# zhanglei1172/sam-quantization

Hardware: AMD Instinct MI355X
Metric: 1024×1024 images/sec through quantized ViT-H encoder; % of MFMA/HBM roofline (higher is better)
Workload: dtype fp16

## Files before the change

### sam-quantization_amd/csrc/attention.hip

```cpp
#include "common.h"

#include <cstdio>
#include <cstdlib>
#include <algorithm>
#include <string>
#include <type_traits>
#include <vector>

namespace samq {

constexpr float LOG2E = 1.4426950408889634f;

__device__ __attribute__((aligned(16))) _Float16 g_zero16[8];

struct AttnParams {
  const _Float16* qkv;
  const _Float16* qkv_bias;
  const _Float16* relh;
  const _Float16* relw;
  _Float16* out;
  int64_t tok_stride;
  int C, heads;
  int S;
  int H, W;
// ... 100 lines not shown
    const _Float16* src = g_zero16;
    bool real = false;
    if (c < UNIT_CHUNKS) {
      constexpr int HALF = UNIT_CHUNKS / 2;
      const bool isv = c >= HALF;
      const int cc = isv ? c - HALF : c;
      const int key = cc / D8, d8 = cc % D8;
      const int r = RESIDENT ? key / S : 0;
      const int slot = RESIDENT ? key % S : key;
      const int kind = r < S ? tok_kind(r, slot) : 2;
      const int off = (isv ? 2 * C : C) + head * D + d8 * 8;
      if (kind == 0) { src = tok_ptr(r, slot) + off; real = true; }
      else if (kind == 1 && p.qkv_bias) src = p.qkv_bias + off;
    }
    src0[i] = src;
    adv[i] = real && !RESIDENT;
  }
  const int64_t rowstride = (int64_t)p.W * p.tok_stride;
  auto issue = [&](int row0, int buf) {
#pragma unroll
    for (int i = 0; i < NI; ++i) {
      const _Float16* src = adv[i] ? src0[i] + row0 * rowstride : src0[i];
      __builtin_amdgcn_global_load_lds((const SAMQ_GLOBAL void*)src,
                                       (SAMQ_LDS void*)(smem + buf * BUFB + (wave * NI + i) * 1024), 16, 0, 0);
    }
  };

  issue(0, 0);
  if (!RESIDENT && S > 1) issue(1, 1);

  const bool kin3 = 64 + 8 * g < D;
  half8_t qf[QT][KS];
  int qrow[QT], qcol0[QT];
#pragma unroll
  for (int t = 0; t < QT; ++t) {
    const int qi = (qblk * NW + wave) * QT + t;
    qrow[t] = qi / KT;
    qcol0[t] = (qi % KT) * 16;
    const int kind = tok_kind(qrow[t], qcol0[t] + ql);
    const _Float16* src = nullptr;
    if (kind == 0) src = tok_ptr(qrow[t], qcol0[t] + ql) + head * D;
    else if (kind == 1 && p.qkv_bias) src = p.qkv_bias + head * D;
#pragma unroll
    for (int s = 0; s < KS; ++s) {
      half8_t v = {};
      if (src && (s < 2 || kin3)) v = *(const half8_t*)(src + 32 * s + 8 * g);
#pragma unroll
      for (int j = 0; j < 8; ++j) v[j] = (_Float16)((float)v[j] * qscale);
      qf[t][s] = v;
    }
  }

  float4_t tw[QT][KT];
  const float inv_scale = 1.0f / p.scale;
  float* th_w = th_lds + wave * (QT * TH_ROWS * 16);
#pragma unroll
  for (int t = 0; t < QT; ++t) {
    const int qh = qrow[t] < S ? qrow[t] : S - 1;
    if (!PRECOMP) {
#pragma unroll
      for (int which = 0; which < 2; ++which) {
        const _Float16* tab = which ? p.relw : p.relh;
#pragma unroll
        for (int kt = 0; kt < KT; ++kt) {
          int r = qh - (kt * 16 + ql) + S - 1;
          r = r < 0 ? 0 : r;
          const _Float16* rp = tab + (int64_t)r * D;
          float4_t a = {0.f, 0.f, 0.f, 0.f};
#pragma unroll
          for (int s = 0; s < KS; ++s) {
            half8_t ra = {};
            if (s < 2 || kin3) ra = *(const half8_t*)(rp + 32 * s + 8 * g);
            a = __builtin_amdgcn_mfma_f32_16x16x32_f16(ra, qf[t][s], a, 0, 0, 0);
          }
          a = a * inv_scale;
          if (which) {
            tw[t][kt] = a;
          } else {
#pragma unroll
            for (int r2 = 0; r2 < 4; ++r2) th_w[(t * TH_ROWS + kt * 16 + 4 * g + r2) * 16 + ql] = a[r2];
          }
        }
      }
    } else {
      const int qw = qcol0[t] + ql;
      const bool ok = qw < S && qrow[t] < S;
      const int64_t base = ((((int64_t)unit * p.heads + head) * S + qh) * S + (ok ? qw : 0)) * S;
#pragma unroll
      for (int kt = 0; kt < KT; ++kt) {
#pragma unroll
        for (int r2 = 0; r2 < 4; ++r2) {
          const int kk = kt * 16 + 4 * g + r2;
          const bool kin = ok && kk < S;
          tw[t][kt][r2] = kin ? (float)p.relw[base + kk] * LOG2E : 0.f;
          th_w[(t * TH_ROWS + kk) * 16 + ql] = kin ? (float)p.relh[base + kk] * LOG2E : 0.f;
        }
      }
    }
  }

  constexpr bool MSUM = SP >= 32;
  float m[QT], l[QT];
  float4_t o[QT][DT], lacc[QT];
  const half8_t ones = {1, 1, 1, 1, 1, 1, 1, 1};
#pragma unroll
  for (int t = 0; t < QT; ++t) {
    m[t] = -INFINITY;
    l[t] = 0.f;
    lacc[t] = float4_t{0.f, 0.f, 0.f, 0.f};
#pragma unroll
    for (int d = 0; d < DT; ++d) o[t][d] = float4_t{0.f, 0.f, 0.f, 0.f};
  }
  const bool mask_slots = S < SP;
  const int trow = ql >> 2;
  const int tcol = 4 * (ql & 3);

  if (RESIDENT) {
    wait_vmcnt<0>();
    __syncthreads();
  } else {
    __syncthreads();
  }

  using PB = half8_t[QT][(SP + 31) / 32];
  auto qk = [&](const char* kb, float4_t (&sc)[QT][KT]) {
#pragma unroll
      for (int kt = 0; kt < KT; ++kt) {
        const char* krow = kb + (kt * 16 + ql) * (D * 2);
        half8_t kf[KS];
#pragma unroll
        for (int s = 0; s < KS; ++s) kf[s] = *(const half8_t*)(krow + (32 * s + 8 * g) * 2);
#pragma unroll
        for (int t = 0; t < QT; ++t) {
          float4_t a = tw[t][kt];
#pragma unroll
          for (int s = 0; s < KS; ++s) a = __builtin_amdgcn_mfma_f32_16x16x32_f16(kf[s], qf[t][s], a, 0, 0, 0);
          sc[t][kt] = a;
        }
      }

  };
  auto soft = [&](int kh, float4_t (&sc)[QT][KT], PB& pb, half4_t (&pb16)[QT]) {
    bool any_rescale = false;
    float alpha[QT];
#pragma unroll
    for (int t = 0; t < QT; ++t) {
      if (mask_slots) {
#pragma unroll
        for (int kt = 0; kt < KT; ++kt)
#pragma unroll
          for (int r = 0; r < 4; ++r)
            if (kt * 16 + 4 * g + r >= S) sc[t][kt][r] = -INFINITY;
      }
      float mx;
      if constexpr (KT == 1) {
        mx = max3f(sc[t][0][0], sc[t][0][1], fmaxf(sc[t][0][2], sc[t][0][3]));
      } else {
        mx = max3f(sc[t][0][0], sc[t][0][1], sc[t][0][2]);
        float my = max3f(sc[t][1][0], sc[t][1][1], sc[t][1][2]);
        mx = max3f(mx, sc[t][0][3], sc[t][1][3]);
#pragma unroll
        for (int kt = 2; kt < KT; kt += 2) {
          mx = max3f(mx, sc[t][kt][0], sc[t][kt][1]);
          my = max3f(my, sc[t][kt + 1][0], sc[t][kt + 1][1]);
          mx = max3f(mx, sc[t][kt][2], sc[t][kt][3]);
          my = max3f(my, sc[t][kt + 1][2], sc[t][kt + 1][3]);
        }
        mx = fmaxf(mx, my);
      }
      mx = max_rows4(mx);
      const float th = th_w[(t * TH_ROWS + kh) * 16 + ql];
      const float mrow = mx + th;
      const bool up = mrow > m[t] + 8.0f;
      const float mnew = up ? mrow : m[t];
      alpha[t] = up ? __builtin_amdgcn_exp2f(m[t] - mnew) : 1.0f;
      any_rescale |= up;
      m[t] = mnew;
      const float corr = mnew - th;
      float rs = 0.f;
#pragma unroll
      for (int kt = 0; kt < KT; ++kt)
#pragma unroll
        for (int r = 0; r < 4; ++r) {
          const float e = __builtin_amdgcn_exp2f(sc[t][kt][r] - corr);
          sc[t][kt][r] = e;
          if (!MSUM) rs += e;
        }
      if (!MSUM) l[t] = l[t] * alpha[t] + rs;
      if (SP == 16) {
        pb16[t] = half4_t{(_Float16)sc[t][0][0], (_Float16)sc[t][0][1], (_Float16)sc[t][0][2], (_Float16)sc[t][0][3]};
      } else {
#pragma unroll
        for (int s = 0; s < SP / 32; ++s) {
#pragma unroll
          for (int r = 0; r < 4; ++r) {
            pb[t][s][r] = (_Float16)sc[t][2 * s][r];
            pb[t][s][4 + r] = (_Float16)sc[t][2 * s + 1][r];
          }
        }
      }
    }
    if (__any(any_rescale)) {
#pragma unroll
      for (int t = 0; t < QT; ++t)
#pragma unroll
        for (int d = 0; d < DT; ++d) o[t][d] = o[t][d] * alpha[t];
#pragma unroll
      for (int t = 0; t < QT; ++t)
        if (MSUM) lacc[t] = lacc[t] * alpha[t];
    }

  };
  auto pv = [&](const char* vb, PB& pb, half4_t (&pb16)[QT]) {
    const uint32_t vbase = lds_addr(vb + ((4 * g + trow) * D + tcol) * 2);
    static_for<DT>([&](auto dc_) {
      constexpr int d = decltype(dc_)::value;
      if constexpr (SP == 16) {
        half4_t va = ds_read_tr16_off<(d * 16) * 2>(vbase);
        asm volatile("s_waitcnt lgkmcnt(0)" : "+v"(va));
#pragma unroll
        for (int t = 0; t < QT; ++t) o[t][d] = __builtin_amdgcn_mfma_f32_16x16x16f16(va, pb16[t], o[t][d], 0, 0, 0);
      } else {
        constexpr int NS = SP / 32;
        half4_t lo[NS], hi[NS];
        static_for<NS>([&](auto sc_) {
          constexpr int s_ = decltype(sc_)::value;
          lo[s_] = ds_read_tr16_off<((32 * s_) * D + d * 16) * 2>(vbase);
          hi[s_] = ds_read_tr16_off<((32 * s_ + 16) * D + d * 16) * 2>(vbase);
        });
        if constexpr (NS == 2) {
          asm volatile("s_waitcnt lgkmcnt(0)" : "+v"(lo[0]), "+v"(hi[0]), "+v"(lo[1]), "+v"(hi[1]));
        } else {
#pragma unroll
          for (int s = 0; s < NS; ++s) asm volatile("s_waitcnt lgkmcnt(0)" : "+v"(lo[s]), "+v"(hi[s]));
        }
#pragma unroll
        for (int s = 0; s < NS; ++s) {
          const half8_t va = {lo[s][0], lo[s][1], lo[s][2], lo[s][3], hi[s][0], hi[s][1], hi[s][2], hi[s][3]};
#pragma unroll
          for (int t = 0; t < QT; ++t) o[t][d] = __builtin_amdgcn_mfma_f32_16x16x32_f16(va, pb[t][s], o[t][d], 0, 0, 0);
        }
      }
    });
    if constexpr (MSUM) {
      constexpr int NS = SP / 32;
#pragma unroll
      for (int s = 0; s < NS; ++s)
#pragma unroll
        for (int t = 0; t < QT; ++t) lacc[t] = __builtin_amdgcn_mfma_f32_16x16x32_f16(ones, pb[t][s], lacc[t], 0, 0, 0);
    }
  };

  if (RESIDENT) {
    for (int kh = 0; kh < S; ++kh) {
      const char* kb = smem + kh * S * (D * 2);
      float4_t sc[QT][KT];
      PB pb;
      half4_t pb16[QT];
      qk(kb, sc);
      soft(kh, sc, pb, pb16);
      pv(kb + (UNIT_CHUNKS / 2) * 16, pb, pb16);
    }
  } else {
    float4_t scA[QT][KT], scB[QT][KT];
    PB pb;
    half4_t pb16[QT];
    if (S > 1) wait_vmcnt<NI>(); else wait_vmcnt<0>();
    __builtin_amdgcn_s_barrier();
    qk(smem, scA);
    auto step = [&](int kh, float4_t (&cur)[QT][KT], float4_t (&nxt)[QT][KT]) {
      if (kh + 1 < S) {
        wait_vmcnt<0>();
        __builtin_amdgcn_s_barrier();
        if (kh + 2 < S) issue(kh + 2, (kh + 2) % 3);
        qk(smem + ((kh + 1) % 3) * BUFB, nxt);
      }
      soft(kh, cur, pb, pb16);
      pv(smem + (kh % 3) * BUFB + ROWB, pb, pb16);
    };
    for (int kh = 0; kh < S; kh += 2) {
      step(kh, scA, scB);
      step(kh + 1, scB, scA);
    }
  }

#pragma unroll
  for (int t = 0; t < QT; ++t) {
    float lt = l[t];
    if (MSUM) {
      lt = lacc[t][0];
    } else {
      lt += __shfl_xor(lt, 16, 64);
      lt += __shfl_xor(lt, 32, 64);
    }
    const int x = qcol0[t] + ql;
    if (tok_kind(qrow[t], x) != 0) continue;
    const float inv = 1.0f / lt;
    const int64_t dst = (((int64_t)b * p.H + (Y0 + qrow[t])) * p.W + (X0 + x)) * C + head * D;
#pragma unroll
    for (int d = 0; d < DT; ++d) attn_store4(p, dst + d * 16 + 4 * g, o[t][d] * inv);
  }
}

template <int D, bool UNSC = false, bool PHL = false>
struct Win {
  static constexpr int S = 14, QT = 2;
  static constexpr int KS = D == 80 ? 3 : 2;
  static constexpr int DT = D / 16;
  static constexpr int NPC = D == 80 ? 5 : 4;
  static constexpr int ROWB = NPC * 1024;
  static constexpr int KVB = S * ROWB;
  static constexpr int V0 = (NPC - 2) * 1024;
  static constexpr int TAB = (2 * S - 1) * D;
  static constexpr int TABB = ((2 * TAB * 2 + 1023) / 1024) * 1024;
  static_assert(D == 64 || D == 80, "head dim");

  struct Geo { const _Float16* tok0; int b, Y0, X0, head, nrow, ncol; };

  __device__ static __forceinline__ Geo geo(const AttnParams& p, int item) {
    Geo o;
    const int unit = item / p.heads;
    o.head = item - unit * p.heads;
    o.b = unit / p.upi;
    const int wi = unit - o.b * p.upi;
    const int wy = wi / p.nwx;
    o.Y0 = wy * S;
    o.X0 = (wi - wy * p.nwx) * S;
    o.nrow = p.H - o.Y0 < S ? p.H - o.Y0 : S;
    o.ncol = p.W - o.X0 < S ? p.W - o.X0 : S;
    o.tok0 = p.qkv + (((int64_t)o.b * p.H + o.Y0) * p.W + o.X0) * p.tok_stride;
    return o;
  }

  __device__ static __forceinline__ void issue_tables(const AttnParams& p, char* tab, int lane, int i0, int istep) {
    for (int i = i0; i < TABB / 1024; i += istep) {
      const int c = i * 64 + lane;
      const int tc = c < TAB / 8 ? c : c - TAB / 8;
      const _Float16* src = c < 2 * (TAB / 8) ? (c < TAB / 8 ? p.relh : p.relw) + 8 * tc : g_zero16;
      __builtin_amdgcn_global_load_lds((const SAMQ_GLOBAL void*)src, (SAMQ_LDS void*)(tab + i * 1024), 16, 0, 0);
    }
  }

  __device__ static __forceinline__ void issue_rows(const AttnParams& p, const Geo& G, char* kv, int lane, int kh0,
                                                    int khstep) {
    const int ql = lane & 15, g = lane >> 4;
    const int64_t ts = p.tok_stride, rowstride = (int64_t)p.W * ts;
    const _Float16* src[NPC];
    int64_t step[NPC];
    const _Float16* pad[NPC];
#pragma unroll
    for (int j = 0; j < NPC; ++j) {
      int col, ch;
      if (j < KS - (D == 80 ? 1 : 0) || (D == 80 && j == 2 && lane < 32)) {
        col = ql;
        ch = p.C + G.head * D + 32 * j + 8 * g;
      } else {
        const bool comb = D == 80 && j == 2;
        const int g8 = comb ? g - 2 : g;
        const int dblk = comb ? 2 : j - (NPC - 2);
        col = ql ^ (8 * (g8 & 1));
        ch = 2 * p.C + G.head * D + 32 * dblk + 8 * g8;
      }
      col = col < S - 1 ? col : S - 1;
      pad[j] = p.qkv_bias ? p.qkv_bias + ch : g_zero16;
      const bool real = col < G.ncol;
      src[j] = real ? G.tok0 + (int64_t)col * ts + ch + kh0 * rowstride : pad[j];
      step[j] = real ? khstep * rowstride : 0;
    }
    for (int kh = kh0; kh < S; kh += khstep) {
      const bool rowreal = kh < G.nrow;
#pragma unroll
      for (int j = 0; j < NPC; ++j) {
        __builtin_amdgcn_global_load_lds((const SAMQ_GLOBAL void*)(rowreal ? src[j] : pad[j]),
                                         (SAMQ_LDS void*)(kv + kh * ROWB + j * 1024), 16, 0, 0);
        src[j] += step[j];
      }
    }
  }

  __device__ static __forceinline__ void load_q(const AttnParams& p, const Geo& G, int r, int lane, half8_t (&q)[KS]) {
    const int ql = lane & 15, g = lane >> 4;
    const bool inwin = ql < S && r < S;
    const bool real = inwin && r < G.nrow && ql < G.ncol;
    const _Float16* base = real ? G.tok0 + ((int64_t)r * p.W + ql) * p.tok_stride + G.head * D
                                : ((inwin && p.qkv_bias) ? p.qkv_bias + G.head * D : nullptr);
#pragma unroll
    for (int s = 0; s < KS; ++s) {
      const _Float16* a = (base && 32 * s + 8 * g < D) ? base + 32 * s + 8 * g : g_zero16;
      asm volatile("" : "+v"(a));
      q[s] = *(const SAMQ_GLOBAL half8_t*)a;
    }
  }

  template <typename F>
  __device__ static __forceinline__ void tiles(const AttnParams& p, const Geo& G, const char* kv, const char* tab,
                                               half8_t (&qraw)[QT][KS], int row0, int lane, F&& after_qk) {
    const int ql = lane & 15, g = lane >> 4;
    const float qscale = p.scale * LOG2E;
    const float inv_scale = 1.0f / p.scale;
    const _Float16* tabh = (const _Float16*)tab;
    half8_t relh[QT][KS], relw[QT][KS];
#pragma unroll
    for (int t = 0; t < QT; ++t) {
      int idx = row0 + t - ql + S - 1;
      idx = idx < 0 ? 0 : idx;
#pragma unroll
      for (int s = 0; s < KS; ++s) {
        int dd = 32 * s + 8 * g;
        dd = dd < D ? dd : dd - 16;
        relh[t][s] = *(const half8_t*)(tabh + idx * D + dd);
        relw[t][s] = *(const half8_t*)(tabh + TAB + idx * D + dd);
      }
    }
    half8_t qf[QT][KS];
    float4_t tw[QT];
    half8_t th[QT][2];
#pragma unroll
    for (int t = 0; t < QT; ++t) {
#pragma unroll
      for (int s = 0; s < KS; ++s) {
        half8_t v = qraw[t][s];
        if constexpr (!UNSC) {
#pragma unroll
          for (int j = 0; j < 8; ++j) v[j] = (_Float16)__builtin_fmaf((float)v[j], qscale, 0.0f);
        }
        qf[t][s] = v;
      }
      float4_t a = {0.f, 0.f, 0.f, 0.f}, c = {0.f, 0.f, 0.f, 0.f};
#pragma unroll
      for (int s = 0; s < KS; ++s) {
        a = __builtin_amdgcn_mfma_f32_16x16x32_f16(relw[t][s], qf[t][s], a, 0, 0, 0);
        c = __builtin_amdgcn_mfma_f32_16x16x32_f16(relh[t][s], qf[t][s], c, 0, 0, 0);
      }
      a = a * inv_scale;
      if constexpr (!UNSC) c = c * inv_scale;
      if (g == 3) { a[2] = -INFINITY; a[3] = -INFINITY; }
      tw[t] = a;
      union { half4_t h; uint32_t u[2]; } mine;
      mine.h = half4_t{(_Float16)c[0], (_Float16)c[1], (_Float16)c[2], (_Float16)c[3]};
      union { half8_t h[2]; uint32_t u[8]; } all;
#pragma unroll
      for (int gg = 0; gg < 4; ++gg)
#pragma unroll
        for (int w = 0; w < 2; ++w) all.u[2 * gg + w] = (uint32_t)__shfl((int)mine.u[w], ql + 16 * gg, 64);
      th[t][0] = all.h[0];
      th[t][1] = all.h[1];
    }

    float4_t sc[QT][S];
    half8_t kf[2][KS];
#pragma unroll
    for (int s = 0; s < KS; ++s) kf[0][s] = *(const half8_t*)(kv + s * 1024 + lane * 16);
#pragma unroll
    for (int kh = 0; kh < S; ++kh) {
      if (kh + 1 < S) {
#pragma unroll
        for (int s = 0; s < KS; ++s) kf[(kh + 1) & 1][s] = *(const half8_t*)(kv + (kh + 1) * ROWB + s * 1024 + lane * 16);
      }
#pragma unroll
      for (int t = 0; t < QT; ++t) {
        const float h = UNSC ? (float)th[t][kh >> 3][kh & 7] * inv_scale : (float)th[t][kh >> 3][kh & 7];
        float4_t a = tw[t] + h;
#pragma unroll
        for (int s = 0; s < KS; ++s) a = __builtin_amdgcn_mfma_f32_16x16x32_f16(kf[kh & 1][s], qf[t][s], a, 0, 0, 0);
        sc[t][kh] = a;
      }
      __builtin_amdgcn_sched_barrier(0);
    }
    after_qk();

    half8_t pb[QT][S / 2];
    half8_t pl[PHL ? QT : 1][PHL ? S / 2 : 1];
#pragma unroll
    for (int t = 0; t < QT; ++t) {
      float mx = max3f(sc[t][0][0], sc[t][0][1], sc[t][0][2]);
      float my = max3f(sc[t][1][0], sc[t][1][1], sc[t][1][2]);
      mx = max3f(mx, sc[t][0][3], sc[t][1][3]);
#pragma unroll
      for (int kh = 2; kh < S; kh += 2) {
        mx = max3f(mx, sc[t][kh][0], sc[t][kh][1]);
        my = max3f(my, sc[t][kh + 1][0], sc[t][kh + 1][1]);
        mx = max3f(mx, sc[t][kh][2], sc[t][kh][3]);
        my = max3f(my, sc[t][kh + 1][2], sc[t][kh + 1][3]);
      }
      mx = fmaxf(mx, my);
      mx = max_rows4(mx);
      if constexpr (UNSC && PHL) {
        const float nmx = -mx * qscale;
#pragma unroll
        for (int pr = 0; pr < S / 2; ++pr)
#pragma unroll
          for (int r = 0; r < 8; ++r) {
            const float e = __builtin_amdgcn_exp2f(__builtin_fmaf(sc[t][2 * pr + (r >> 2)][r & 3], qscale, nmx));
            const _Float16 hi = (_Float16)e;
            pb[t][pr][r] = hi;
            pl[PHL ? t : 0][PHL ? pr : 0][r] = (_Float16)(e - (float)hi);
          }
      } else if constexpr (UNSC) {
        const float nmx = -mx * qscale;
#pragma unroll
        for (int pr = 0; pr < S / 2; ++pr)
#pragma unroll
          for (int r = 0; r < 4; ++r) {
            pb[t][pr][r] = (_Float16)__builtin_amdgcn_exp2f(__builtin_fmaf(sc[t][2 * pr][r], qscale, nmx));
            pb[t][pr][4 + r] = (_Float16)__builtin_amdgcn_exp2f(__builtin_fmaf(sc[t][2 * pr + 1][r], qscale, nmx));
          }
      } else {
#pragma unroll
        for (int pr = 0; pr < S / 2; ++pr)
#pragma unroll
          for (int r = 0; r < 4; ++r) {
            pb[t][pr][r] = (_Float16)__builtin_amdgcn_exp2f(sc[t][2 * pr][r] - mx);
            pb[t][pr][4 + r] = (_Float16)__builtin_amdgcn_exp2f(sc[t][2 * pr + 1][r] - mx);
          }
      }
    }

    const int tq = ql >> 2, tp = ql & 3;
    const int vslot = 4 * g + tq;
    const uint32_t vlane = lds_addr(kv) + (((tp >> 1) * 16 + (vslot ^ (8 * (tp >> 1)))) * 16 + (tp & 1) * 8);
    const half8_t ones = {1, 1, 1, 1, 1, 1, 1, 1};
    float4_t o[QT][DT], lsum[QT];
    const float4_t zero4 = {0.f, 0.f, 0.f, 0.f};
    half4_t vlo[2][DT], vhi[2][DT];
    auto vread = [&](auto prc, half4_t (&lo)[DT], half4_t (&hi)[DT]) {
      constexpr int PR = decltype(prc)::value;
      constexpr int HB = PR >= 4 ? 32768 : 0;
      const uint32_t base = vlane + HB;
      static_for<DT>([&](auto dc) {
        constexpr int d = decltype(dc)::value;
        constexpr int VO = d < 4 ? V0 + (d >> 1) * 1024 + (d & 1) * 512 : 2 * 1024 + 512;
        lo[d] = ds_read_tr16_off<(2 * PR) * ROWB + VO - HB>(base);
        hi[d] = ds_read_tr16_off<(2 * PR + 1) * ROWB + VO - HB>(base);
      });
    };
    vread(std::integral_constant<int, 0>{}, vlo[0], vhi[0]);
    static_for<S / 2>([&](auto prc) {
      constexpr int pr = decltype(prc)::value;
      constexpr int cb = pr & 1;
      if constexpr (pr + 1 < S / 2) vread(std::integral_constant<int, pr + 1>{}, vlo[cb ^ 1], vhi[cb ^ 1]);
      if constexpr (DT == 5) {
        if (pr + 1 < S / 2)
          asm volatile("s_waitcnt lgkmcnt(10)" : "+v"(vlo[cb][0]), "+v"(vlo[cb][1]), "+v"(vlo[cb][2]), "+v"(vlo[cb][3]),
                       "+v"(vlo[cb][4]), "+v"(vhi[cb][0]), "+v"(vhi[cb][1]), "+v"(vhi[cb][2]), "+v"(vhi[cb][3]), "+v"(vhi[cb][4]));
        else
          asm volatile("s_waitcnt lgkmcnt(0)" : "+v"(vlo[cb][0]), "+v"(vlo[cb][1]), "+v"(vlo[cb][2]), "+v"(vlo[cb][3]),
                       "+v"(vlo[cb][4]), "+v"(vhi[cb][0]), "+v"(vhi[cb][1]), "+v"(vhi[cb][2]), "+v"(vhi[cb][3]), "+v"(vhi[cb][4]));
      } else {
        if (pr + 1 < S / 2)
          asm volatile("s_waitcnt lgkmcnt(8)" : "+v"(vlo[cb][0]), "+v"(vlo[cb][1]), "+v"(vlo[cb][2]), "+v"(vlo[cb][3]),
                       "+v"(vhi[cb][0]), "+v"(vhi[cb][1]), "+v"(vhi[cb][2]), "+v"(vhi[cb][3]));
        else
          asm volatile("s_waitcnt lgkmcnt(0)" : "+v"(vlo[cb][0]), "+v"(vlo[cb][1]), "+v"(vlo[cb][2]), "+v"(vlo[cb][3]),
                       "+v"(vhi[cb][0]), "+v"(vhi[cb][1]), "+v"(vhi[cb][2]), "+v"(vhi[cb][3]));
      }
#pragma unroll
      for (int d = 0; d < DT; ++d) {
        const half8_t va = {vlo[cb][d][0], vlo[cb][d][1], vlo[cb][d][2], vlo[cb][d][3],
                            vhi[cb][d][0], vhi[cb][d][1], vhi[cb][d][2], vhi[cb][d][3]};
#pragma unroll
        for (int t = 0; t < QT; ++t) {
          o[t][d] = __builtin_amdgcn_mfma_f32_16x16x32_f16(va, pb[t][pr], pr ? o[t][d] : zero4, 0, 0, 0);
          if constexpr (PHL) o[t][d] = __builtin_amdgcn_mfma_f32_16x16x32_f16(va, pl[t][pr], o[t][d], 0, 0, 0);
        }
      }
#pragma unroll
      for (int t = 0; t < QT; ++t) {
        lsum[t] = __builtin_amdgcn_mfma_f32_16x16x32_f16(ones, pb[t][pr], pr ? lsum[t] : zero4, 0, 0, 0);
        if constexpr (PHL) lsum[t] = __builtin_amdgcn_mfma_f32_16x16x32_f16(ones, pl[t][pr], lsum[t], 0, 0, 0);
      }
    });

#pragma unroll
    for (int t = 0; t < QT; ++t) {
      const int r = row0 + t;
      if (r >= G.nrow || ql >= G.ncol) continue;
      const float inv = __builtin_amdgcn_rcpf(lsum[t][0]);
      const int64_t dst = (((int64_t)G.b * p.H + (G.Y0 + r)) * p.W + (G.X0 + ql)) * p.C + G.head * D;
#pragma unroll
      for (int d = 0; d < DT; ++d) attn_store4(p, dst + d * 16 + 4 * g, o[t][d] * inv);
    }
  }
};

template <int D, bool UNSC = false, bool PHL = false>
__global__ __launch_bounds__(256, 2) void win_attention_kernel(AttnParams p, int items) {
  using W = Win<D, UNSC, PHL>;
  static_assert(W::KVB + W::TABB <= 80 * 1024, "two workgroups per CU");
  __shared__ __attribute__((aligned(16))) char smem[W::KVB + W::TABB];
  const int lane = threadIdx.x & 63, wave = threadIdx.x >> 6;
  const int item = xcd_remap(blockIdx.x, gridDim.x);
  if (item >= items) return;
  const typename W::Geo G = W::geo(p, item);
  char* tab = smem + W::KVB;
  W::issue_tables(p, tab, lane, wave, 4);
  W::issue_rows(p, G, smem, lane, wave, 4);
  half8_t qraw[W::QT][W::KS];
#pragma unroll
  for (int t = 0; t < W::QT; ++t) W::load_q(p, G, 2 * wave + t, lane, qraw[t]);
  wait_vmcnt<0>();
  __syncthreads();
  const int npass = 8 + 2 * wave < W::S ? 2 : 1;
  for (int pass = 0; pass < npass; ++pass) {
    const int row0 = 8 * pass + 2 * wave;
    W::tiles(p, G, smem, tab, qraw, row0, lane, [&] {
      if (pass + 1 < npass) {
#pragma unroll
        for (int t = 0; t < W::QT; ++t) W::load_q(p, G, row0 + 8 + t, lane, qraw[t]);
      }
    });
  }
}

__device__ __forceinline__ float16_t mfma32(half8_t a, half8_t b, float16_t c) {
  return __builtin_amdgcn_mfma_f32_32x32x16_f16(a, b, c, 0, 0, 0);
}

#ifdef SAMQ_TUNING
__device__ unsigned long long g_attn_stamps[8];
__device__ unsigned long long g_attn_wgt[4096 * 6];
#endif
template <int DBG>
__device__ __forceinline__ void wg_mark(unsigned long long (&t)[6], int k) {
  if constexpr ((DBG & 8) != 0) {
    t[k] = __builtin_amdgcn_s_memrealtime();
    if (k == 1 || k == 2) t[k + 3] = __builtin_amdgcn_s_memtime();
  }
}

template <int DBG>
__global__ __launch_bounds__(512, 1) void glob80_attention_kernel(AttnParams p) {
  constexpr int D = 80, S = 64, KS = 5;
  constexpr int NSLOT = 5;
  constexpr bool ONESL = (DBG & 512) == 0;
  constexpr int VB = 10 * 1024;
  constexpr int V2B = 18 * 1024;
  constexpr int ONESB = V2B + 2048 + 128;
  constexpr int ROWB = ONESL ? ONESB + 2048 : 20 * 1024;
  constexpr int THB = 64 * 32 * 2;
  __shared__ __attribute__((aligned(16))) char smem[NSLOT * ROWB + 8 * THB];
  static_assert(NSLOT * ROWB + 8 * THB <= 160 * 1024, "LDS");
  constexpr bool DBG_NOEXP = (DBG & 2) != 0, DBG_NOMFMA = (DBG & 4) != 0;
  constexpr bool COFF = (DBG & 16) == 0;
  constexpr bool KEARLY = (DBG & 32) != 0, VPRE = (DBG & 64) != 0, PFENCE = (DBG & 128) == 0;
  constexpr bool CMFMA = (DBG & 256) != 0 && COFF;
  constexpr bool G1DMA = (DBG & 1024) != 0;
  constexpr bool STATPRIO = (DBG & 2048) != 0;
  constexpr bool QKDMA = (DBG & 4096) != 0;

  _Float16* th_lds = (_Float16*)(smem + NSLOT * ROWB);
  unsigned long long wgt[6] = {0, 0, 0, 0, 0, 0};
  wg_mark<DBG>(wgt, 0);

  const int tid = threadIdx.x;
  const int lane = tid & 63;
  const int wave = __builtin_amdgcn_readfirstlane(tid >> 6);
  const int grp = wave >> 2;
  const int l32 = lane & 31, h = lane >> 5;
  const int nqb = p.nqb, pairs = p.heads * p.units;
  const int xcd = blockIdx.x & 7, kk = blockIdx.x >> 3;
  const int pair = xcd * (pairs >> 3) + kk / nqb;
  const int qblk = kk % nqb;
  const int head = pair % p.heads;
  const int b = pair / p.heads;
  const int C = p.C;
  const int qh = 4 * qblk + (wave >> 1);
  const int qw0 = 32 * (wave & 1);
  const _Float16* img = p.qkv + (int64_t)b * S * S * p.tok_stride;

  constexpr int NI = G1DMA ? 5 : 3;
  const int npc = G1DMA ? (grp ? 5 : 0) : (wave < 4 ? 3 : 2);
  const _Float16* src0[NI];
  int dst[NI];
#pragma unroll
  for (int i = 0; i < NI; ++i) {
    const int v = G1DMA ? (wave & 3) + 4 * i : wave + 8 * i;
    int key, dim;
    if (v < 10) {
      key = 32 * (v / 5) + l32;
      dim = C + 16 * (v % 5) + 8 * h;
    } else if (ONESL) {
      const int gl = 64 * (v - 10) + lane;
      if (v < 18) {
        const int kq = gl >> 5, w = gl & 31;
        key = 4 * kq + ((w & 15) >> 2);
        dim = 2 * C + 32 * (w >> 4) + 8 * (w & 3);
      } else {
        const int g2 = gl - 512, kq = g2 >> 3, w = g2 & 7;
        key = 4 * kq + (w >> 1);
        dim = 2 * C + 64 + 8 * (w & 1);
      }
      key = key < S ? key : S - 1;
    } else {
      const int gl = 64 * (v - 10) + lane;
      const int kq = gl / 40, w = gl % 40;
      if (w < 16)      { key = 4 * kq + (w >> 2);        dim = 2 * C + 8 * (w & 3); }
      else if (w < 32) { key = 4 * kq + ((w - 16) >> 2); dim = 2 * C + 32 + 8 * (w & 3); }
      else             { key = 4 * kq + ((w - 32) >> 1); dim = 2 * C + 64 + 8 * (w & 1); }
      key = key < S ? key : S - 1;
    }
    src0[i] = img + (int64_t)key * p.tok_stride + head * D + dim;
    dst[i] = v * 1024;
  }
  const int64_t rowstride = (int64_t)S * p.tok_stride;
  auto issue_one = [&](int kh, int slot, int i) {
    if (i < npc)
      __builtin_amdgcn_global_load_lds((const SAMQ_GLOBAL void*)(src0[i] + kh * rowstride),
                                       (SAMQ_LDS void*)(smem + slot * ROWB + dst[i]), 16, 0, 0);
  };
  auto issue = [&](int kh, int slot) {
#pragma unroll
    for (int i = 0; i < NI; ++i) issue_one(kh, slot, i);
  };
#pragma unroll
  for (int r = 0; r < NSLOT - 1; ++r) issue(r, r);

  const float qscale = p.scale * LOG2E;
  half8_t qf[KS];
  {
    const _Float16* qp = img + ((int64_t)qh * S + qw0 + l32) * p.tok_stride + head * D + 8 * h;
#pragma unroll
    for (int s = 0; s < KS; ++s) {
      half8_t v = *(const half8_t*)(qp + 16 * s);
#pragma unroll
      for (int j = 0; j < 8; ++j) v[j] = (_Float16)__builtin_fmaf((float)v[j], qscale, 0.0f);
      qf[s] = v;
    }
  }
  const float inv_scale = 1.0f / p.scale;
  float16_t tw[2];
  _Float16* thw = th_lds + wave * (64 * 32);
#pragma unroll
  for (int which = 0; which < 2; ++which) {
    const _Float16* tab = which ? p.relw : p.relh;
#pragma unroll
    for (int kt = 0; kt < 2; ++kt) {
      const int r = qh - (32 * kt + l32) + S - 1;
      const _Float16* rp = tab + (int64_t)r * D + 8 * h;
      float16_t a = {};
#pragma unroll
      for (int s = 0; s < KS; ++s) a = mfma32(*(const half8_t*)(rp + 16 * s), qf[s], a);
      a = a * inv_scale;
      if (which) {
        tw[kt] = a;
      } else {
#pragma unroll
        for (int r2 = 0; r2 < 16; ++r2) {
          const int kh = 32 * kt + 8 * (r2 >> 2) + 4 * h + (r2 & 3);
          thw[kh * 32 + l32] = (_Float16)a[r2];
        }
      }
    }
  }

  const int i16 = lane & 15, g16 = (lane >> 4) & 1;
  const int tq = i16 >> 2, tp = i16 & 3;
  constexpr int QB = ONESL ? 512 : 640, QB2 = ONESL ? 128 : 640;
  const uint32_t vb01 = lds_addr(smem + VB) + h * QB + tq * 64 + g16 * 32 + tp * 8;
  const uint32_t vb2 = ONESL ? lds_addr(smem + V2B) + h * QB2 + tq * 32 + tp * 8 + g16 * (ONESB - V2B)
                             : lds_addr(smem + VB) + h * 640 + 512 + tq * 32 + tp * 8;
  const uint32_t ones_or = g16 ? 0x3C003C00u : 0u, ones_and = g16 ? 0u : 0xFFFFFFFFu;
  if constexpr (ONESL) {
    const u32x4 one4 = {0x3C003C00u, 0x3C003C00u, 0x3C003C00u, 0x3C003C00u};
    for (int i = tid; i < NSLOT * 128; i += 512)
      *(u32x4*)(smem + (i >> 7) * ROWB + ONESB + (i & 127) * 16) = one4;
  }

  float16_t o[3];
#pragma unroll
  for (int d = 0; d < 3; ++d) o[d] = float16_t{};
  float m = -INFINITY;
  float16_t sc[2];
  half8_t pb[2][2];

  half8_t kf[2][KS];
  auto kread = [&](const char* kb) {
#pragma unroll
    for (int kt = 0; kt < 2; ++kt)
#pragma unroll
      for (int s = 0; s < KS; ++s) kf[kt][s] = *(const half8_t*)(kb + (kt * 5 + s) * 1024 + lane * 16);
  };
  float coff = 0.f;
  const half8_t ones01 = h ? half8_t{} : half8_t{1, 1, 0, 0, 0, 0, 0, 0};
  half8_t cq = {};
  auto set_cq = [&] {
    const _Float16 hi = (_Float16)coff;
    const _Float16 lo = (_Float16)(coff - (float)hi);
    cq = h ? half8_t{} : half8_t{hi, lo, 0, 0, 0, 0, 0, 0};
  };
  auto qk_d = [&](auto&& dma) {
#pragma unroll
    for (int kt = 0; kt < 2; ++kt) {
      float16_t a = tw[kt];
      if constexpr (CMFMA) a = mfma32(ones01, cq, a);
      else if constexpr (COFF) a = a + coff;
#pragma unroll
      for (int s = 0; s < KS; ++s) {
        if (DBG_NOMFMA) a[s] += (float)kf[kt][s][0] * (float)qf[s][0];
        else a = mfma32(kf[kt][s], qf[s], a);
        dma(KS * kt + s);
      }
      sc[kt] = a;
    }
  };
  auto qk = [&]() { qk_d([](int) {}); };
  float th_cur = (float)thw[l32];
  float m_pend = -INFINITY;
  bool pend = false;
  float moff = 0.f;
  if constexpr (COFF) coff = th_cur;
  if constexpr (CMFMA) set_cq();
  auto softmax_coff = [&](int kh) {
    if (__any(pend)) {
      const float alpha = pend ? __builtin_amdgcn_exp2f(m - m_pend) : 1.0f;
      m = pend ? m_pend : m;
#pragma unroll
      for (int d = 0; d < 3; ++d) o[d] = o[d] * alpha;
      pend = false;
    }
#pragma unroll
    for (int kt = 0; kt < 2; ++kt)
#pragma unroll
      for (int u = 0; u < 2; ++u)
#pragma unroll
        for (int j = 0; j < 8; ++j) pb[kt][u][j] = (_Float16)__builtin_amdgcn_exp2f(sc[kt][8 * u + j]);
    if constexpr (PFENCE) asm volatile("" : "+v"(pb[0][0]), "+v"(pb[0][1]), "+v"(pb[1][0]), "+v"(pb[1][1]));
    float mx = max3f(sc[0][0], sc[0][1], sc[0][2]);
    float my = max3f(sc[1][0], sc[1][1], sc[1][2]);
#pragma unroll
    for (int r = 3; r + 1 < 16; r += 2) {
      mx = max3f(mx, sc[0][r], sc[0][r + 1]);
      my = max3f(my, sc[1][r], sc[1][r + 1]);
    }
    mx = max3f(mx, my, fmaxf(sc[0][15], sc[1][15]));
    {
      const auto sw = __builtin_amdgcn_permlane32_swap(__builtin_bit_cast(int, mx), __builtin_bit_cast(int, mx),
                                                       false, false);
      mx = fmaxf(__builtin_bit_cast(float, (int)sw[0]), __builtin_bit_cast(float, (int)sw[1]));
    }
    const float mrow = mx + moff;
    const bool unsafe = !(mrow <= m + 15.0f);
    if (__any(unsafe)) {
      const float mnew = unsafe ? mrow : m;
      const float alpha = unsafe ? __builtin_amdgcn_exp2f(m - mnew) : 1.0f;
      m = mnew;
#pragma unroll
      for (int d = 0; d < 3; ++d) o[d] = o[d] * alpha;
      const float delta = m - moff;
#pragma unroll
      for (int kt = 0; kt < 2; ++kt)
#pragma unroll
        for (int u = 0; u < 2; ++u)
#pragma unroll
          for (int j = 0; j < 8; ++j) pb[kt][u][j] = (_Float16)__builtin_amdgcn_exp2f(sc[kt][8 * u + j] - delta);
    }
    pend = mrow > m + 8.0f;
    m_pend = mrow;
    if (kh + 1 < S) {
      th_cur = (float)thw[(kh + 1) * 32 + l32];
      moff = pend ? m_pend : m;
      coff = th_cur - moff;
      if constexpr (CMFMA) set_cq();
    }
  };
  auto softmax = [&](int kh) {
    if constexpr (COFF) return softmax_coff(kh);
    if (__any(pend)) {
      const float alpha = pend ? __builtin_amdgcn_exp2f(m - m_pend) : 1.0f;
      m = pend ? m_pend : m;
#pragma unroll
      for (int d = 0; d < 3; ++d) o[d] = o[d] * alpha;
      pend = false;
    }
    float corr = m - th_cur;
#pragma unroll
    for (int kt = 0; kt < 2; ++kt)
#pragma unroll
      for (int u = 0; u < 2; ++u)
#pragma unroll
        for (int j = 0; j < 8; ++j) pb[kt][u][j] = (_Float16)(DBG_NOEXP ? sc[kt][8 * u + j] - corr
                                                                   : __builtin_amdgcn_exp2f(sc[kt][8 * u + j] - corr));
    float mx = max3f(sc[0][0], sc[0][1], sc[0][2]);
    float my = max3f(sc[1][0], sc[1][1], sc[1][2]);
#pragma unroll
    for (int r = 3; r + 1 < 16; r += 2) {
      mx = max3f(mx, sc[0][r], sc[0][r + 1]);
      my = max3f(my, sc[1][r], sc[1][r + 1]);
    }
    mx = max3f(mx, my, fmaxf(sc[0][15], sc[1][15]));
    {
      const auto sw = __builtin_amdgcn_permlane32_swap(__builtin_bit_cast(int, mx), __builtin_bit_cast(int, mx),
                                                       false, false);
      mx = fmaxf(__builtin_bit_cast(float, (int)sw[0]), __builtin_bit_cast(float, (int)sw[1]));
    }
    const float mrow = mx + th_cur;
    const bool unsafe = !(mrow <= m + 15.0f);
    if (__any(unsafe)) {
      const float mnew = unsafe ? mrow : m;
      const float alpha = unsafe ? __builtin_amdgcn_exp2f(m - mnew) : 1.0f;
      m = mnew;
#pragma unroll
      for (int d = 0; d < 3; ++d) o[d] = o[d] * alpha;
      corr = m - th_cur;
#pragma unroll
      for (int kt = 0; kt < 2; ++kt)
#pragma unroll
        for (int u = 0; u < 2; ++u)
#pragma unroll
// ... 421 lines not shown
```

Measured before the change: 179.6.

## Pack narrow edge windows two rows per tile and balance window scheduling across XCDs

Adds a decoder that orders window/head items so full-size and partial edge windows are spread evenly over the 8 XCDs, replacing the plain xcd_remap. For edge windows whose width is at most 8 columns, two query rows are packed into one 16-lane MFMA tile, roughly halving the QK/PV work for those windows. Waves with no valid rows now skip their passes. This cuts wasted MFMA work on padded edge windows and evens out per-XCD load, at the cost of more index arithmetic and an extra code path that doubles the relative-position MFMAs for packed tiles.

```diff
diff --git a/sam-quantization_amd/csrc/attention.hip b/sam-quantization_amd/csrc/attention.hip
--- a/sam-quantization_amd/csrc/attention.hip
+++ b/sam-quantization_amd/csrc/attention.hip
@@ -426,6 +426,42 @@
   }
 }
 
+struct WinItem { int b, wy, wx, head; };
+__host__ __device__ inline WinItem win_decode(int bid, int images, int heads, int nwy, int nwx, int H, int W,
+                                              int S) {
+  const int ly = nwy - (H - (nwy - 1) * S <= 8 ? 1 : 0);
+  const int lx = nwx - (W - (nwx - 1) * S <= 8 ? 1 : 0);
+  const int LW = ly * lx, SW = nwy * nwx - LW;
+  const int nl = images * LW * heads, ns = images * SW * heads;
+  const int ql = nl >> 3, rl = nl & 7, qs = ns >> 3, rs = ns & 7;
+  const int x = bid & 7, k = bid >> 3;
+  const int cl = ql + (x < rl ? 1 : 0);
+  int unit, wy, wx;
+  WinItem o;
+  if (k < cl) {
+    const int i = x * ql + (x < rl ? x : rl) + k;
+    unit = i / heads;
+    o.head = i - unit * heads;
+    o.b = unit / LW;
+    const int wl = unit - o.b * LW;
+    wy = wl / lx;
+    wx = wl - wy * lx;
+  } else {
+    const int xs = (x - rl) & 7;
+    const int i = xs * qs + (xs < rs ? xs : rs) + (k - cl);
+    unit = i / heads;
+    o.head = i - unit * heads;
+    o.b = unit / SW;
+    const int ws = unit - o.b * SW;
+    const int ncolw = ly * (nwx - lx);
+    wy = ws < ncolw ? ws : ly;
+    wx = ws < ncolw ? lx : ws - ncolw;
+  }
+  o.wy = wy;
+  o.wx = wx;
+  return o;
+}
+
 template <int D, bool UNSC = false, bool PHL = false>
 struct Win {
   static constexpr int S = 14, QT = 2;
@@ -441,15 +477,13 @@
 
   struct Geo { const _Float16* tok0; int b, Y0, X0, head, nrow, ncol; };
 
-  __device__ static __forceinline__ Geo geo(const AttnParams& p, int item) {
+  __device__ static __forceinline__ Geo geo(const AttnParams& p, int bid, int items) {
     Geo o;
-    const int unit = item / p.heads;
-    o.head = item - unit * p.heads;
-    o.b = unit / p.upi;
-    const int wi = unit - o.b * p.upi;
-    const int wy = wi / p.nwx;
-    o.Y0 = wy * S;
-    o.X0 = (wi - wy * p.nwx) * S;
+    const WinItem it = win_decode(bid, items / (p.upi * p.heads), p.heads, p.upi / p.nwx, p.nwx, p.H, p.W, S);
+    o.head = it.head;
+    o.b = it.b;
+    o.Y0 = it.wy * S;
+    o.X0 = it.wx * S;
     o.nrow = p.H - o.Y0 < S ? p.H - o.Y0 : S;
     o.ncol = p.W - o.X0 < S ? p.W - o.X0 : S;
     o.tok0 = p.qkv + (((int64_t)o.b * p.H + o.Y0) * p.W + o.X0) * p.tok_stride;
@@ -502,8 +536,11 @@
     }
   }
 
-  __device__ static __forceinline__ void load_q(const AttnParams& p, const Geo& G, int r, int lane, half8_t (&q)[KS]) {
-    const int ql = lane & 15, g = lane >> 4;
+  template <bool PK = false>
+  __device__ static __forceinline__ void load_q(const AttnParams& p, const Geo& G, int r0, int lane, half8_t (&q)[KS]) {
+    const int g = lane >> 4;
+    const int r = PK ? r0 + ((lane >> 3) & 1) : r0;
+    const int ql = PK ? lane & 7 : lane & 15;
     const bool inwin = ql < S && r < S;
     const bool real = inwin && r < G.nrow && ql < G.ncol;
     const _Float16* base = real ? G.tok0 + ((int64_t)r * p.W + ql) * p.tok_stride + G.head * D
@@ -516,18 +553,20 @@
     }
   }
 
-  template <typename F>
+  template <bool PK, typename F>
   __device__ static __forceinline__ void tiles(const AttnParams& p, const Geo& G, const char* kv, const char* tab,
                                                half8_t (&qraw)[QT][KS], int row0, int lane, F&& after_qk) {
     const int ql = lane & 15, g = lane >> 4;
     const float qscale = p.scale * LOG2E;
     const float inv_scale = 1.0f / p.scale;
     const _Float16* tabh = (const _Float16*)tab;
-    half8_t relh[QT][KS], relw[QT][KS];
-#pragma unroll
-    for (int t = 0; t < QT; ++t) {
+    constexpr int NR = PK ? 2 * QT : QT;
+    half8_t relh[NR][KS], relw[NR][KS];
+#pragma unroll
+    for (int t = 0; t < NR; ++t) {
       int idx = row0 + t - ql + S - 1;
       idx = idx < 0 ? 0 : idx;
+      if constexpr (PK) idx = idx > 2 * S - 2 ? 2 * S - 2 : idx;
 #pragma unroll
       for (int s = 0; s < KS; ++s) {
         int dd = 32 * s + 8 * g;
@@ -551,10 +590,26 @@
         qf[t][s] = v;
       }
       float4_t a = {0.f, 0.f, 0.f, 0.f}, c = {0.f, 0.f, 0.f, 0.f};
-#pragma unroll
-      for (int s = 0; s < KS; ++s) {
-        a = __builtin_amdgcn_mfma_f32_16x16x32_f16(relw[t][s], qf[t][s], a, 0, 0, 0);
-        c = __builtin_amdgcn_mfma_f32_16x16x32_f16(relh[t][s], qf[t][s], c, 0, 0, 0);
+      if constexpr (PK) {
+        float4_t a1 = a, c1 = c;
+#pragma unroll
+        for (int s = 0; s < KS; ++s) {
+          a = __builtin_amdgcn_mfma_f32_16x16x32_f16(relw[2 * t][s], qf[t][s], a, 0, 0, 0);
+          c = __builtin_amdgcn_mfma_f32_16x16x32_f16(relh[2 * t][s], qf[t][s], c, 0, 0, 0);
+          a1 = __builtin_amdgcn_mfma_f32_16x16x32_f16(relw[2 * t + 1][s], qf[t][s], a1, 0, 0, 0);
+          c1 = __builtin_amdgcn_mfma_f32_16x16x32_f16(relh[2 * t + 1][s], qf[t][s], c1, 0, 0, 0);
+        }
+#pragma unroll
+        for (int j = 0; j < 4; ++j) {
+          a[j] = ql < 8 ? a[j] : a1[j];
+          c[j] = ql < 8 ? c[j] : c1[j];
+        }
+      } else {
+#pragma unroll
+        for (int s = 0; s < KS; ++s) {
+          a = __builtin_amdgcn_mfma_f32_16x16x32_f16(relw[t][s], qf[t][s], a, 0, 0, 0);
+          c = __builtin_amdgcn_mfma_f32_16x16x32_f16(relh[t][s], qf[t][s], c, 0, 0, 0);
+        }
       }
       a = a * inv_scale;
       if constexpr (!UNSC) c = c * inv_scale;
@@ -697,10 +752,11 @@
 
 #pragma unroll
     for (int t = 0; t < QT; ++t) {
-      const int r = row0 + t;
-      if (r >= G.nrow || ql >= G.ncol) continue;
+      const int r = PK ? row0 + 2 * t + (ql >> 3) : row0 + t;
+      const int qc = PK ? ql & 7 : ql;
+      if (r >= G.nrow || qc >= G.ncol) continue;
       const float inv = __builtin_amdgcn_rcpf(lsum[t][0]);
-      const int64_t dst = (((int64_t)G.b * p.H + (G.Y0 + r)) * p.W + (G.X0 + ql)) * p.C + G.head * D;
+      const int64_t dst = (((int64_t)G.b * p.H + (G.Y0 + r)) * p.W + (G.X0 + qc)) * p.C + G.head * D;
 #pragma unroll
       for (int d = 0; d < DT; ++d) attn_store4(p, dst + d * 16 + 4 * g, o[t][d] * inv);
     }
@@ -712,22 +768,34 @@
   using W = Win<D, UNSC, PHL>;
   static_assert(W::KVB + W::TABB <= 80 * 1024, "two workgroups per CU");
   __shared__ __attribute__((aligned(16))) char smem[W::KVB + W::TABB];
-  const int lane = threadIdx.x & 63, wave = threadIdx.x >> 6;
-  const int item = xcd_remap(blockIdx.x, gridDim.x);
-  if (item >= items) return;
-  const typename W::Geo G = W::geo(p, item);
+  const int lane = threadIdx.x & 63, wave = __builtin_amdgcn_readfirstlane(threadIdx.x >> 6);
+  if ((int)blockIdx.x >= items) return;
+  const typename W::Geo G = W::geo(p, blockIdx.x, items);
   char* tab = smem + W::KVB;
+  const bool packed = G.ncol <= 8;
+  const int npass = packed ? (4 * wave < G.nrow ? 1 : 0) : (2 * wave < G.nrow ? 1 : 0) + (8 + 2 * wave < G.nrow ? 1 : 0);
   W::issue_tables(p, tab, lane, wave, 4);
   W::issue_rows(p, G, smem, lane, wave, 4);
   half8_t qraw[W::QT][W::KS];
-#pragma unroll
-  for (int t = 0; t < W::QT; ++t) W::load_q(p, G, 2 * wave + t, lane, qraw[t]);
+  if (packed) {
+    if (npass) {
+#pragma unroll
+      for (int t = 0; t < W::QT; ++t) W::template load_q<true>(p, G, 4 * wave + 2 * t, lane, qraw[t]);
+    }
+    wait_vmcnt<0>();
+    __syncthreads();
+    if (npass) W::template tiles<true>(p, G, smem, tab, qraw, 4 * wave, lane, [] {});
+    return;
+  }
+  if (npass) {
+#pragma unroll
+    for (int t = 0; t < W::QT; ++t) W::load_q(p, G, 2 * wave + t, lane, qraw[t]);
+  }
   wait_vmcnt<0>();
   __syncthreads();
-  const int npass = 8 + 2 * wave < W::S ? 2 : 1;
   for (int pass = 0; pass < npass; ++pass) {
     const int row0 = 8 * pass + 2 * wave;
-    W::tiles(p, G, smem, tab, qraw, row0, lane, [&] {
+    W::template tiles<false>(p, G, smem, tab, qraw, row0, lane, [&] {
       if (pass + 1 < npass) {
 #pragma unroll
         for (int t = 0; t < W::QT; ++t) W::load_q(p, G, row0 + 8 + t, lane, qraw[t]);
```

Result: no change. 180.5, median of 6 (+0.5%).
